# marcowus/forging-control

Hardware: AMD Instinct MI355X
Metric: rollout-steps/s (batch x horizon), fwd+bwd+AdamW step (higher is better)
Workload: dtype f32

## Files before the change

### forging-control_amd/csrc/fcr_common.h

```cpp
#pragma once
#include <hip/hip_runtime.h>
#include <stddef.h>
#include <stdint.h>

namespace fcr {

typedef float f32x4 __attribute__((ext_vector_type(4)));
typedef float f32x2 __attribute__((ext_vector_type(2)));

constexpr int kWave = 64;
constexpr int kTile = 16;
constexpr int kL = 10;
constexpr int kLayers = 3;
constexpr int kIn = 5;
constexpr int kOut = 4;
constexpr int kCtrlIn = 3;
constexpr int kMS = 13;
constexpr int kFnpStride = 8;
constexpr int kFwdWaves = 8;
constexpr int kBwdWaves = 8;
constexpr float kP1Max = 2.122366f;
constexpr float kP2Max = 1.036233f;

template <int HS>
// ... 9 lines not shown
    const float *fcb;
    const float *fnp;
    const float *wsc;
};

struct FwdArgs {
    int B, N;
    float alpha;
    const float *X, *u0, *states, *noise;
    float *cost, *command, *error, *prediction, *xhat_user, *xhat_ws, *loss_part;
    f32x4 *hseq;
    f32x4 *cseq;
    f32x2 *xw;
    unsigned long long *stamp;
    Packed p;
};

struct BwdArgs {
    int B, N, hidden;
    float alpha;
    const float *X, *states, *prediction, *xhat, *dloss;
    const f32x4 *hseq, *cseq;
    const f32x2 *xw;
    f32x4 *dseq;
    f32x2 *dxrow;
    float *g_u0;
    float *dv;
    unsigned long long *stamp;
    Packed p;
};
// ... 251 lines not shown
    return xor_sum_q(part);
}

__device__ __forceinline__ void grad_out5(float *part, int hidden, int k, int p, float s, float *gwi, float *gbi,
                                          float *gwo) {
    if (gwi) {
        const float v = 0.0f + s;
        if (p < 3) gwi[k * kCtrlIn + p] = v;
        else if (p == 3) gbi[k] = v;
        else gwo[k] = v;
    } else {
        part[((size_t)blockIdx.x * hidden + k) * 5 + p] = s;
    }
}

}
```

### forging-control_amd/csrc/fcr_f16.h

```cpp
#pragma once
#include "fcr_common.h"
#include "fcr_pack.h"

namespace fcr {

typedef _Float16 f16x8 __attribute__((ext_vector_type(8)));

__host__ __device__ constexpr bool tail_packed(int HS) { return 2 * HS - 8 * ((2 * HS + 7) / 8 - 1) == 2; }

template <int HS>
struct Geo16 {
    static constexpr int KB0 = (HS + 2 + 7) / 8;
    static constexpr int XBLK = HS >> 3;
    static constexpr int KB1 = (2 * HS + 7) / 8;
    static constexpr int KX1 = (HS + 7) / 8;
    static constexpr bool TAIL1 = tail_packed(HS);
    static constexpr int QF0 = HS * KB0 * 2;
    static constexpr int QH1 = HS * KB1;
    static constexpr int QF1 = QH1 + HS * (KB1 - (TAIL1 ? 1 : 0));
    static constexpr int FA0 = QF0 * kWave * 4, FA1 = QF1 * kWave * 4, FH1 = QH1 * kWave * 4;
    static constexpr int FNP = kMS * 4 * kFnpStride;
    static constexpr int FCP = kOut * HS * 4;
    static constexpr int MISC = FNP + FCP + 4;
    static constexpr int LDS_FWD = (FA1 + FA0 + MISC) * 4;
// ... 297 lines not shown
    const float d_o = 1.0f + __builtin_amdgcn_exp2f(__builtin_amdgcn_fmed3f(a[3], -1e30f, 126.0f));
    const float o = __builtin_amdgcn_rcpf(d_o);
    const float gi = g * i;
    const float cf = FIRST ? 0.0f : f * c_prev;
    const float tc = h * d_o;
    P = f32x4{fmaf(-h, tc, o), fmaf(-h, o, h), fmaf(-gi, i, gi), fmaf(-cf, f, cf)};
    Q = f32x2{fmaf(-gi, g, i), f};
}

inline size_t f16_fwd_bytes(int HS, int l) {
    const int KB = l == 0 ? (HS + 2 + 7) / 8 : (2 * HS + 7) / 8;
    const int lo_blocks = (l > 0 && tail_packed(HS)) ? KB - 1 : KB;
    return (size_t)HS * (KB + lo_blocks) * kWave * 16;
}

__device__ __forceinline__ float fwd16_weight(const PackArgs &a, int l, int unit, int gate, int s, int kq) {
    const int H = a.H, HS = a.HS;
    float v = 0.0f;
    if (unit < H) {
        const int grow = gate * H + unit;
        if (l == 0) {
            if (s < HS) {
                const int u = 4 * s + kq;
                if (u < H) v = a.whh[0][grow * H + u];
            } else if (s == HS) {
                v = a.wih[0][grow * kIn + kq] / a.wsc[kq];
            } else if (s == HS + 1 && kq == 0) {
                v = a.wih[0][grow * kIn + 4] / a.wsc[4];
            }
        } else if (s < HS) {
            const int u = 4 * s + kq;
            if (u < H) v = a.wih[l][grow * H + u];
        } else if (s < 2 * HS) {
            const int u = 4 * (s - HS) + kq;
            if (u < H) v = a.whh[l][grow * H + u];
        }
    }
    return v * (gate == 2 ? kTwoLog2e : kNegLog2e);
}

__device__ __forceinline__ void pack_fwd16_item(const PackArgs &a, int l, _Float16 *dst, int idx) {
    const int HS = a.HS;
    const int KB = l == 0 ? (HS + 2 + 7) / 8 : (2 * HS + 7) / 8;
    const bool tail = l > 0 && tail_packed(HS);
    const int KL = tail ? KB - 1 : KB;
    const int n = HS * KB * kWave * 8;
    if (idx >= n) return;
    const int j = idx & 7, lane = (idx >> 3) & 63, rk = idx >> 9;
    const int kb = rk % KB, r = rk / KB;
    const int rho = lane & 15, kq = lane >> 4;
    const int unit = 4 * r + (rho >> 2), gate = rho & 3;
    if (tail && kb == KB - 1) {
        _Float16 out = (_Float16)0.0f;
        if (j < 6) {
            const float v = fwd16_weight(a, l, unit, gate, 8 * kb + (j & 1), kq);
            const _Float16 hi = (_Float16)v;
            out = (j == 2 || j == 3) ? (_Float16)(v - (float)hi) : hi;
        }
        dst[((size_t)rk * kWave + lane) * 8 + j] = out;
        return;
    }
    const float v = fwd16_weight(a, l, unit, gate, 8 * kb + j, kq);
    const _Float16 hi = (_Float16)v;
    const _Float16 lo = (_Float16)(v - (float)hi);
    const size_t nq = (size_t)HS * KB;
    dst[((size_t)rk * kWave + lane) * 8 + j] = hi;
    dst[((nq + (size_t)r * KL + kb) * kWave + lane) * 8 + j] = lo;
}

}
```

### forging-control_amd/csrc/fcr_fwd.h

```cpp
#pragma once
#include "fcr_common.h"
#include "fcr_f16.h"

namespace fcr {

__device__ __forceinline__ void rot_left(float (&w)[kL]) {
    const float t0 = w[0];
#pragma unroll
    for (int k = 0; k < kL - 1; ++k) w[k] = w[k + 1];
    w[kL - 1] = t0;
}

struct Pace {
    unsigned turn;
};
__device__ __forceinline__ void pace_cell(Pace &p) {
    if (p.turn & 1) __builtin_amdgcn_s_setprio(1);
    else __builtin_amdgcn_s_setprio(0);
    p.turn ^= 1;
}

template <int HS, bool L0, bool FIRST, bool LP, int R0 = 0, int R1 = HS>
__device__ __forceinline__ void fwd16_cell(const float *__restrict__ lw, int lane, float x0, float x1,
                                           const float (&x)[HS], const float (&hp)[HS], float (&c)[HS],
// ... 293 lines not shown
        const float err = sq(xh0 - ref);
        const float con = relu(-xh1) + relu(-xh2) + relu(xh1 - kP1Max) + relu(xh2 - kP2Max);
        tot_sum += (err + cmd_j) + con;
        err_sum += err;
        cmd_sum += cmd_j;
    }
    const float cost = tot_sum / (float)N;
    if (valid && q == 0) {
        a.cost[b] = cost;
        a.command[b] = cmd_sum / (float)N;
        a.error[b] = err_sum / (float)N;
    }
    float part = (valid && q == 0) ? cost : 0.0f;
#pragma unroll
    for (int m = 1; m < 64; m <<= 1) part += __shfl_xor(part, m);
    if (lane == 0) a.loss_part[wave] = part;
#if FCR_STAMP
    if (lane == 0) {
        unsigned long long *o = a.stamp + (size_t)wave * 8;
        o[0] = st_head;
        o[1] = st_l0;
        o[2] = st_fill;
        o[3] = st_l2;
        o[4] = fstamp() - st_k0;
        o[5] = o[6] = o[7] = 0;
    }
#endif
}

}
```

### forging-control_amd/csrc/fcr_host.h

```cpp
#pragma once
#include <hip/hip_runtime.h>
#include <stdint.h>

#include <atomic>

#include "fcr.h"
#include "fcr_common.h"

namespace fcr {

int fail(int code, const char *fmt, ...) __attribute__((format(printf, 2, 3)));
int launch_check(const char *what);
int lds_attr(const void *fn, int bytes, std::atomic<unsigned long long> &done, const char *what);
extern std::atomic<int> g_small_max_batch, g_pipe_max_batch, g_pipe_sets;
extern std::atomic<long long> g_wide_keep_budget;

constexpr int kMaxSlots = 13;
constexpr int kMaxWideH = 2048;
inline bool is_wide(const fcr_dims *d) { return d->H > 4 * kMaxSlots; }
inline int slot_tier(int H) { return H <= 16 ? 4 : (H <= 32 ? 8 : 13); }
inline void note_kernels(fcr_options *o, int family) {
    if (o) o->kernels = family;
}

// ... 3 lines not shown
    size_t operator()(size_t bytes) {
        const size_t o = off;
        off += align_up(bytes);
        return o;
    }
};

struct PackedLayout {
    int HS;
    size_t fa[3], img[3], fcp, fcb, fnp, wsc, rng;
};
void take_packed(Arena &take, PackedLayout &P, bool with_backward);
Packed packed_ptrs(const PackedLayout &P, char *base);
int launch_range(const fcr_dims *d, const float *states, const float *u0, const float *noise, const float *fcw,
                 const float *fcb, float *part, float *wsc, hipStream_t s);
int launch_pack_all(const fcr_weights *w, int H, int CH, const PackedLayout &P, bool with_backward, char *base,
                    unsigned *clear, int nclear, hipStream_t s);
int launch_pack_ctrl(const fcr_weights *w, int CH, float *fcp, float *fcbo, float *fnp, hipStream_t s);
int launch_loss_reduce(const float *part, int n, int B, float *loss, hipStream_t s);
int launch_ctrl_grads(const fcr_dims *d, const float *X, const float *xhat, const float *dv, const float *fnp, float *part,
                      int ctrl_blocks, float *g_w_inp, float *g_b_inp, float *g_w_out, hipStream_t s);
int launch_grad_reduce(const float *part, int blocks, int hidden, float *g_w_inp, float *g_b_inp, float *g_w_out,
                       hipStream_t s);
int launch_grad_reduce_many(const float *part, int blocks, int hidden, int n_models, float *g_w_inp, float *g_b_inp,
                            float *g_w_out, hipStream_t s);
int pipe_max_sets();
size_t rollout_workspace(const fcr_dims *d, int with_backward);
int rollout_forward(const fcr_dims *d, fcr_options *opts, const fcr_weights *w, const float *X, const float *u0,
                    const float *states, const float *noise, float *loss, float *cost, float *command, float *error,
                    float *prediction, float *xhat, int with_backward, char *base, hipStream_t s);
int rollout_backward(const fcr_dims *d, fcr_options *opts, const float *X, const float *states, const float *prediction,
                     const float *dloss, float *g_u0, float *g_w_inp, float *g_b_inp, float *g_w_out, char *base,
// ... 41 lines not shown
```

### forging-control_amd/csrc/fcr_img.h

```cpp
#pragma once
#include "fcr_common.h"
#include "fcr_f16.h"
#include "fcr_pack.h"

namespace fcr {

__host__ __device__ constexpr int img_units(int kb) { return kb > 2 ? 32 : 16; }
__host__ __device__ constexpr int img_tile_units(int U) { return U == 32 ? 536 : 268; }
__host__ __device__ constexpr int img_row_start(int m, int U) {
    return U == 32 ? 33 * m + (m >= 8 ? 8 : 0)
                   : 33 * (m % 4 + 4 * (m / 8)) + (m >= 8 ? 4 : 0) + 16 * ((m / 4) % 2);
}
__host__ __device__ constexpr int img_unit(int kb, int q, int h0, int U) { return q * (U / 4) + 2 * kb + h0; }

template <int HS, bool L0>
struct Img {
    static constexpr int NSL = L0 ? HS + 2 : 2 * HS;
    static constexpr int KB = (NSL + 7) / 8;
    static constexpr int U = img_units(KB);
    static constexpr int TILE = 8 * img_tile_units(U);
    static constexpr int HALF = HS * TILE;
    static constexpr int BYTES = (2 * HALF + 1023) / 1024 * 1024;
    static constexpr int NB = (NSL + 3) / 4;
    static constexpr int KBB = (HS + 1) / 2;
};

inline int img_kb(int HS, int l) { return ((l == 0 ? HS + 2 : 2 * HS) + 7) / 8; }
inline size_t img_bytes(int HS, int l) {
    const int U = img_units(img_kb(HS, l));
    return ((size_t)2 * HS * 8 * img_tile_units(U) + 1023) / 1024 * 1024;
}
inline int img_pack_threads(int HS, int l) { return 16 * HS * 4 * img_units(img_kb(HS, l)); }

__device__ __forceinline__ void pack_img_item(const PackArgs &a, int l, _Float16 *dst, int idx) {
    const int H = a.H, HS = a.HS;
    const int nsl = l == 0 ? HS + 2 : 2 * HS;
    const int kbn = (nsl + 7) / 8;
    const int U = img_units(kbn), TU = img_tile_units(U);
    const int cols = 4 * U, rows = 16 * HS;
    if (idx >= rows * cols) return;
    const int col = idx % cols, R = idx / cols;
    const int slot = R >> 4, m = R & 15;
    const int unit = 4 * slot + (m >> 2), gate = m & 3;
    const int sg = (col >> 5) * 8 + (col & 7), grp = (col >> 3) & 3;
    auto weight = [&](int s) {
        float v = 0.0f;
        if (unit < H && s < nsl) {
            const int grow = gate * H + unit;
            if (l == 0) {
                if (s < HS) {
                    const int u = 4 * s + grp;
                    if (u < H) v = a.whh[0][grow * H + u];
                } else if (s == HS) {
                    v = a.wih[0][grow * kIn + grp] / a.wsc[grp];
                } else if (grp == 0) {
                    v = a.wih[0][grow * kIn + 4] / a.wsc[4];
                }
            } else if (s < HS) {
                const int u = 4 * s + grp;
                if (u < H) v = a.wih[l][grow * H + u];
            } else {
                const int u = 4 * (s - HS) + grp;
                if (u < H) v = a.whh[l][grow * H + u];
            }
        }
        return v * (gate == 2 ? kTwoLog2e : kNegLog2e);
    };
    _Float16 hi, lo;
    const int jt = sg - 8 * (kbn - 1);
    if (l > 0 && tail_packed(HS) && jt >= 2 && jt < 6) {
        const float v = weight(8 * (kbn - 1) + (jt & 1));
// ... 48 lines not shown
```

### forging-control_amd/csrc/fcr_pack.h

```cpp
#pragma once
#include "fcr_common.h"

namespace fcr {

struct PackArgs {
    int H, HS, CH;
    const float *wih[3], *whh[3], *fcw, *fcb, *cwi, *cbi, *cwo;
    float *fcp, *fcbo, *fnp;
    const float *wsc;
};

constexpr int kRangeBlocks = 128;
constexpr int kRangeThreads = 256;
__device__ __forceinline__ void range_final_wave(const float *__restrict__ part, int nblk,
                                                 const float *__restrict__ fcw, const float *__restrict__ fcb,
                                                 int H, float *wsc, int lane) {
    float mc[kIn];
#pragma unroll
    for (int c = 0; c < kIn; ++c) {
        float m = 0.0f;
        for (int i = lane; i < nblk; i += 64) m = fmaxf(m, part[i * 8 + c]);
#pragma unroll
        for (int o = 32; o > 0; o >>= 1) m = fmaxf(m, __shfl_xor(m, o));
        mc[c] = m;
// ... 14 lines not shown
#pragma unroll
                for (int j = 0; j < 8; ++j) v[j] = w[k + j];
#pragma unroll
                for (int j = 0; j < 8; ++j) s += fabsf(v[j]);
            }
            for (; k < H; ++k) s += fabsf(w[k]);
            m += s;
        } else {
            m = fmaxf(m, 1.0f);
        }
        if (isfinite(m) && m >= 16384.0f) sc = __builtin_amdgcn_ldexpf(1.0f, 14 - __builtin_amdgcn_frexp_expf(m));
    }
    wsc[lane] = sc;
}

__device__ __forceinline__ void pack_misc_item(const PackArgs &a, int idx) {
    const int H = a.H, HS = a.HS;
    const int nfc = kOut * HS * 4;
    if (idx < nfc) {
        const int q = idx & 3, r = (idx >> 2) % HS, o = (idx >> 2) / HS;
        const int u = 4 * r + q;
        a.fcp[idx] = u < H ? a.fcw[o * H + u] : 0.0f;
    }
    if (idx < kOut) a.fcbo[idx] = a.fcb[idx];
    const int nf = kMS * 4 * kFnpStride;
    if (idx < nf) {
        const int p = idx % kFnpStride, q = (idx / kFnpStride) & 3, m = idx / (kFnpStride * 4);
        const int k = 4 * m + q;
        float v = 0.0f;
        if (k < a.CH) {
// ... 13 lines not shown
```

### forging-control_amd/csrc/fcr_rollout.hip

```cpp
#include <hip/hip_runtime.h>
#include <stdint.h>

#include <atomic>

#include "fcr.h"
#include "fcr_bwd.h"
#include "fcr_common.h"
#include "fcr_fwd.h"
#include "fcr_host.h"
#include "fcr_img.h"
#include "fcr_pack.h"
#include "fcr_pipe.h"
#include "fcr_shared_kernels.h"
#include "fcr_small.h"
#include "fcr_sur.h"
#include "fcr_lstm_rollout.h"

namespace fcr {
namespace {

struct Layout : PackedLayout {
    int nw, nw_pad;
    size_t xhat, dv, loss_part, fnn_part, hseq, cseq, xw, dseq, dxrow, stamp, total;
    size_t pipe_flags, pipe_rows;
    int ctrl_blocks;
};

constexpr int kPipeMaxGroups = 32;

Layout make_layout(const fcr_dims *d, int with_backward) {
    Layout L{};
    L.HS = slot_tier(d->H);
    L.nw = (d->B + kTile - 1) / kTile;
    constexpr int kPad = kFwdWaves > kBwdWaves ? kFwdWaves : kBwdWaves;
    L.nw_pad = (L.nw + kPad - 1) / kPad * kPad;
    Arena take;
    const int HS = L.HS;
    take_packed(take, L, with_backward != 0);
    L.xhat = take(sizeof(float) * (size_t)d->B * d->N * kOut);
    L.loss_part = take(sizeof(float) * L.nw_pad);
    L.dv = take(sizeof(float) * (size_t)d->B * d->N);
    L.ctrl_blocks = (int)(((long long)d->B * d->N + kCtrlItems - 1) / kCtrlItems);
    L.fnn_part = take(sizeof(float) * (size_t)L.ctrl_blocks * d->ctrl_hidden * 5);
// ... 132 lines not shown
    hipLaunchKernelGGL((fcr_sbwd_kernel<HS>), dim3(L.nw), dim3(Small<HS>::NQ * kWave), lds, s, ba);
    return launch_check("fcr_sbwd_kernel");
}

enum { kPackFwd16 = 0, kPackImg = 1, kPackMisc = 2 };
struct PackJob {
    int kind, l, blocks;
    _Float16 *dst;
};
struct PackAllArgs {
    PackArgs a;
    int njobs;
    PackJob job[2 * kLayers + 1];
    unsigned *clear;
    int nclear;
};
__global__ __launch_bounds__(256) void pack_all_kernel(PackAllArgs p) {
    if (p.clear && blockIdx.x == 0)
        for (int i = (int)threadIdx.x; i < p.nclear; i += 256) p.clear[i] = 0u;
    int b = blockIdx.x, j = 0;
    while (j + 1 < p.njobs && b >= p.job[j].blocks) b -= p.job[j++].blocks;
    const int idx = b * 256 + (int)threadIdx.x;
    const PackJob &jb = p.job[j];
    if (jb.kind == kPackFwd16) pack_fwd16_item(p.a, jb.l, jb.dst, idx);
    else if (jb.kind == kPackImg) pack_img_item(p.a, jb.l, jb.dst, idx);
    else pack_misc_item(p.a, idx);
}
}

void take_packed(Arena &take, PackedLayout &P, bool with_backward) {
    const int HS = P.HS;
    for (int l = 0; l < kLayers; ++l) P.fa[l] = take(f16_fwd_bytes(HS, l));
    if (with_backward)
        for (int l = 0; l < kLayers; ++l) P.img[l] = take(img_bytes(HS, l));
    P.fcp = take(sizeof(float) * kOut * HS * 4);
    P.fcb = take(sizeof(float) * kOut);
    P.fnp = take(sizeof(float) * kMS * 4 * kFnpStride);
    P.wsc = take(sizeof(float) * 8);
    P.rng = take(sizeof(float) * 8 * kRangeBlocks);
}

int launch_pack_all(const fcr_weights *w, int H, int CH, const PackedLayout &P, bool with_backward, char *base,
                    unsigned *clear, int nclear, hipStream_t s) {
    PackAllArgs pk{};
    PackArgs &pa = pk.a;
    pa.H = H;
    pa.HS = P.HS;
    pa.CH = CH;
    for (int l = 0; l < kLayers; ++l) {
        pa.wih[l] = w->w_ih[l];
        pa.whh[l] = w->w_hh[l];
    }
    pa.fcw = w->fc_w;
    pa.fcb = w->fc_b;
    if (CH) {
        pa.cwi = w->ctrl_w_inp;
        pa.cbi = w->ctrl_b_inp;
        pa.cwo = w->ctrl_w_out;
    }
    pa.fcp = (float *)(base + P.fcp);
    pa.fcbo = (float *)(base + P.fcb);
    pa.fnp = (float *)(base + P.fnp);
    pa.wsc = (const float *)(base + P.wsc);
    pk.clear = clear;
    pk.nclear = nclear;
    for (int l = 0; l < kLayers; ++l) {
        const int nf = P.HS * (l == 0 ? (P.HS + 2 + 7) / 8 : (2 * P.HS + 7) / 8) * kWave * 8;
        pk.job[pk.njobs++] = PackJob{kPackFwd16, l, (nf + 255) / 256, (_Float16 *)(base + P.fa[l])};
        if (with_backward)
            pk.job[pk.njobs++] = PackJob{kPackImg, l, (img_pack_threads(P.HS, l) + 255) / 256, (_Float16 *)(base + P.img[l])};
    }
    pk.job[pk.njobs++] = PackJob{kPackMisc, 0, 2, nullptr};
    int blocks = 0;
    for (int j = 0; j < pk.njobs; ++j) blocks += pk.job[j].blocks;
    hipLaunchKernelGGL(pack_all_kernel, dim3(blocks), dim3(256), 0, s, pk);
    return launch_check("pack_all_kernel");
}

int launch_pack_ctrl(const fcr_weights *w, int CH, float *fcp, float *fcbo, float *fnp, hipStream_t s) {
    PackArgs pa{};
// ... 30 lines not shown
    const size_t rows = (size_t)d->B * (d->N > kL ? d->N : kL);
    if (rows <= 16 * kRangeThreads) {
        hipLaunchKernelGGL(range_partial_kernel, dim3(1), dim3(kRangeThreads), 0, s, states, u0, noise, d->B, d->N,
                           part, fcw, fcb, d->H, wsc);
        return launch_check("range_partial_kernel");
    }
    hipLaunchKernelGGL(range_partial_kernel, dim3(kRangeBlocks), dim3(kRangeThreads), 0, s, states, u0, noise, d->B,
                       d->N, part, nullptr, nullptr, 0, nullptr);
    int rc = launch_check("range_partial_kernel");
    if (rc) return rc;
    hipLaunchKernelGGL(range_final_kernel, dim3(1), dim3(64), 0, s, (const float *)part, kRangeBlocks, fcw, fcb, d->H,
                       wsc);
    return launch_check("range_final_kernel");
}

int launch_ctrl_grads(const fcr_dims *d, const float *X, const float *xhat, const float *dv, const float *fnp, float *part,
                      int ctrl_blocks, float *g_w_inp, float *g_b_inp, float *g_w_out, hipStream_t s) {
    const bool one = ctrl_blocks == 1;
    hipLaunchKernelGGL(ctrl_grad_kernel, dim3(ctrl_blocks), dim3(kCtrlBlock), 0, s, X, xhat, dv, fnp, d->B, d->N,
                       d->ctrl_hidden, part, one ? g_w_inp : nullptr, one ? g_b_inp : nullptr, one ? g_w_out : nullptr);
    if (const int rc = launch_check("ctrl_grad_kernel")) return rc;
    if (one) return FCR_OK;
    return launch_grad_reduce(part, ctrl_blocks, d->ctrl_hidden, g_w_inp, g_b_inp, g_w_out, s);
}

int launch_grad_reduce(const float *part, int blocks, int hidden, float *g_w_inp, float *g_b_inp, float *g_w_out,
                       hipStream_t s) {
    hipLaunchKernelGGL(grad_reduce_kernel, dim3(hidden * 5), dim3(256), 0, s, part, blocks, hidden, g_w_inp, g_b_inp,
                       g_w_out);
    return launch_check("grad_reduce_kernel");
// ... 8 lines not shown
                            float *g_w_out, hipStream_t s) {
    hipLaunchKernelGGL(grad_reduce_many_kernel, dim3(hidden * 5, n_models), dim3(256), 0, s, part, blocks, hidden, g_w_inp,
                       g_b_inp, g_w_out);
    return launch_check("grad_reduce_many_kernel");
}

int pipe_max_sets() { return Pipe<13>::MAX_SETS; }

size_t rollout_workspace(const fcr_dims *d, int with_backward) { return make_layout(d, with_backward).total; }

int rollout_forward(const fcr_dims *d, fcr_options *opts, const fcr_weights *w, const float *X, const float *u0,
                    const float *states, const float *noise, float *loss, float *cost, float *command, float *error,
                    float *prediction, float *xhat, int with_backward, char *base, hipStream_t s) {
    int rc;
    const Layout L = make_layout(d, with_backward);
    if ((rc = launch_range(d, states, u0, noise, w->fc_w, w->fc_b, (float *)(base + L.rng), (float *)(base + L.wsc), s)))
        return rc;
    const bool flags = L.nw <= kPipeMaxGroups;
    if ((rc = launch_pack_all(w, d->H, d->ctrl_hidden, L, with_backward != 0, base,
                              flags ? (unsigned *)(base + L.pipe_flags) : nullptr, flags ? L.nw * kPipeFlags : 0, s)))
        return rc;

    FwdArgs fa{};
    fa.B = d->B;
    fa.N = d->N;
    fa.alpha = d->alpha;
    fa.X = X;
    fa.u0 = u0;
    fa.states = states;
    fa.noise = noise;
    fa.cost = cost;
    fa.command = command;
    fa.error = error;
    fa.prediction = prediction;
    fa.xhat_user = xhat;
    fa.xhat_ws = (float *)(base + L.xhat);
    fa.loss_part = (float *)(base + L.loss_part);
    fa.hseq = (f32x4 *)(base + L.hseq);
    fa.cseq = with_backward ? (f32x4 *)(base + L.cseq) : nullptr;
    fa.xw = with_backward ? (f32x2 *)(base + L.xw) : nullptr;
    fa.p = packed_ptrs(L, base);
#if FCR_STAMP
    fa.stamp = (unsigned long long *)(base + L.stamp) + (size_t)L.nw_pad * 8;
#endif
    const bool small = use_small(d, L, opts);
    note_kernels(opts, small ? FCR_KERNELS_SMALL : FCR_KERNELS_FUSED);
    const bool piped = small && use_pipe(d, L, opts);
    if (piped) {
        PipeArgs pa = pipe_args(L, base);
        pa.loss = loss;
        const int S = pipe_sets(d, L, Pipe<13>::MAX_SETS, 2);
        if (L.HS == 8) rc = with_backward ? launch_pfwd_s<8, true>(fa, pa, L, S, s) : launch_pfwd_s<8, false>(fa, pa, L, S, s);
        else rc = with_backward ? launch_pfwd_s<13, true>(fa, pa, L, S, s) : launch_pfwd_s<13, false>(fa, pa, L, S, s);
    } else if (small) {
        if (L.HS == 8) rc = with_backward ? launch_sfwd_t<8, true>(fa, L, s) : launch_sfwd_t<8, false>(fa, L, s);
        else rc = with_backward ? launch_sfwd_t<13, true>(fa, L, s) : launch_sfwd_t<13, false>(fa, L, s);
    } else {
        switch (L.HS) {
            case 4: rc = launch_fwd<4>(fa, L, d->precision == FCR_PRECISION_F16, s); break;
            case 8: rc = launch_fwd<8>(fa, L, d->precision == FCR_PRECISION_F16, s); break;
            case 13: rc = launch_fwd<13>(fa, L, d->precision == FCR_PRECISION_F16, s); break;
            default: rc = fail(FCR_EUNSUPPORTED, "H=%d", d->H);
        }
    }
    if (rc) return rc;
    if (piped) return FCR_OK;
    return launch_loss_reduce(fa.loss_part, small ? L.nw : L.nw_pad, d->B, loss, s);
}

int rollout_backward(const fcr_dims *d, fcr_options *opts, const float *X, const float *states, const float *prediction,
                     const float *dloss, float *g_u0, float *g_w_inp, float *g_b_inp, float *g_w_out, char *base,
                     hipStream_t s) {
    int rc;
    const Layout L = make_layout(d, 1);
    BwdArgs ba{};
    ba.B = d->B;
    ba.N = d->N;
    ba.hidden = d->ctrl_hidden;
    ba.alpha = d->alpha;
    ba.X = X;
    ba.states = states;
    ba.prediction = prediction;
// ... 89 lines not shown
    const int HS = slot_tier(d->H);
    return !is_wide(d) && (HS == 8 || HS == 13);
}

size_t many_workspace(const fcr_dims *d, int n_models, int with_backward) {
    return make_many(d, n_models, with_backward).total;
}

int many_forward(const fcr_dims *d, int M, const fcr_weights *w, const float *X, const float *u0, const float *states,
                 const float *noise, float *loss, float *cost, float *command, float *error, float *prediction,
                 float *xhat, int with_backward, char *base, hipStream_t s) {
    int rc;
    const ManyLayout L = make_many(d, M, with_backward);
    fcr_dims all = *d;
    all.B = M * d->B;
    if ((rc = launch_range(&all, states, u0, noise, w->fc_w, w->fc_b, (float *)(base + L.rng), (float *)(base + L.wsc), s)))
        return rc;
    if ((rc = launch_pack_all(w, d->H, 0, L, with_backward != 0, base, nullptr, 0, s))) return rc;
    constexpr int nf = kMS * 4 * kFnpStride;
    hipLaunchKernelGGL(pack_fnp_many_kernel, dim3((nf + 255) / 256, M), dim3(256), 0, s, w->ctrl_w_inp, w->ctrl_b_inp,
                       w->ctrl_w_out, d->ctrl_hidden, (float *)(base + L.fnp_many));
    if ((rc = launch_check("pack_fnp_many_kernel"))) return rc;

    FwdArgs fa{};
    fa.B = d->B;
    fa.N = d->N;
    fa.alpha = d->alpha;
    fa.X = X;
    fa.u0 = u0;
    fa.states = states;
    fa.noise = noise;
    fa.cost = cost;
    fa.command = command;
// ... 155 lines not shown
    int rc = launch_check("sur_bwd_kernel");
    if (rc) return rc;
    if ((rc = sur_wgrad_t<HS, false>(a, L, 2, part, g_w_ih[2], g_w_hh[2], s))) return rc;
    if ((rc = sur_wgrad_t<HS, false>(a, L, 1, part, g_w_ih[1], g_w_hh[1], s))) return rc;
    return sur_wgrad_t<HS, true>(a, L, 0, part, g_w_ih[0], g_w_hh[0], s);
}

}

size_t sur_workspace(const fcr_dims *d, int with_backward) { return make_sur(d, with_backward).total; }

int sur_forward(const fcr_dims *d, const fcr_weights *w, const float *x, float *y, int with_backward, char *base,
                hipStream_t s) {
    const SurLayout L = make_sur(d, with_backward);
    int rc;
    if ((rc = launch_range(d, x, x, nullptr, w->fc_w, w->fc_b, (float *)(base + L.rng), (float *)(base + L.wsc), s)))
        return rc;
    if ((rc = launch_pack_all(w, d->H, 0, L, with_backward != 0, base, nullptr, 0, s))) return rc;
    SurArgs a = sur_args(d, L, base);
    a.x = x;
    a.y = y;
    switch (L.HS) {
        case 4: return sur_forward_t<4>(a, L, with_backward != 0, s);
        case 8: return sur_forward_t<8>(a, L, with_backward != 0, s);
        default: return sur_forward_t<13>(a, L, with_backward != 0, s);
    }
}

int sur_backward(const fcr_dims *d, const float *dy, float *const *g_w_ih, float *const *g_w_hh, float *g_fc_w,
                 float *g_fc_b, float *g_x, char *base, hipStream_t s) {
    const SurLayout L = make_sur(d, 1);
    SurArgs a = sur_args(d, L, base);
    a.dy = dy;
// ... 62 lines not shown
    a.g3 = gain ? gain[3] : 1.0f;
    a.xhat = xhat;
    a.hseq = (f32x4 *)(base + L.hseq);
    a.p = packed_ptrs(L, base);
    float *part = (float *)(base + L.rpart), *wsc = (float *)(base + L.wsc);
    const size_t rows = (size_t)d->B * (d->N > kL ? d->N : kL);
    const LroRangeArgs rg{a.g0, a.g1, a.g2, a.g3, w->fc_w, w->fc_b, w->w_ih[0], d->H, wsc};
    const bool one = rows <= 16 * kRangeThreads;
    hipLaunchKernelGGL(lro_range_partial_kernel, dim3(one ? 1 : kRangeBlocks), dim3(kRangeThreads), 0, s, window0, cmd,
                       noise, d->B, d->N, part, one ? 1 : 0, rg);
    if ((rc = launch_check("lro_range_partial_kernel"))) return rc;
    if (!one) {
        hipLaunchKernelGGL(lro_range_final_kernel, dim3(1), dim3(64), 0, s, (const float *)part, kRangeBlocks, rg);
        if ((rc = launch_check("lro_range_final_kernel"))) return rc;
    }
    if ((rc = launch_pack_all(w, d->H, 0, L, false, base, nullptr, 0, s))) return rc;
    switch (L.HS) {
        case 4: return launch_lro_t<4>(a, L, s);
        case 8: return launch_lro_t<8>(a, L, s);
        default: return launch_lro_t<13>(a, L, s);
    }
}

}

#if FCR_STAMP
extern "C" {
size_t fcr_debug_stamp_offset(const fcr_dims *d) { return fcr::make_layout(d, 1).stamp; }
size_t fcr_debug_dseq_offset(const fcr_dims *d) { return fcr::make_layout(d, 1).dseq; }
size_t fcr_debug_dxrow_offset(const fcr_dims *d) { return fcr::make_layout(d, 1).dxrow; }
}
// ... 2 lines not shown
```

### forging-control_amd/csrc/fcr_shared_kernels.h

```cpp
#pragma once
#include "fcr_f16.h"
#include "fcr_img.h"
#include "fcr_pack.h"

namespace fcr {

__global__ __launch_bounds__(64) void range_final_kernel(const float *__restrict__ part, int nblk,
                                                         const float *__restrict__ fcw,
                                                         const float *__restrict__ fcb, int H, float *wsc) {
    range_final_wave(part, nblk, fcw, fcb, H, wsc, threadIdx.x);
}

__global__ __launch_bounds__(kRangeThreads) void range_partial_kernel(const float *__restrict__ states,
                                                                      const float *__restrict__ u0,
                                                                      const float *__restrict__ noise, int B, int N,
                                                                      float *part, const float *fcw = nullptr,
                                                                      const float *fcb = nullptr, int H = 0,
                                                                      float *wsc = nullptr) {
    __shared__ float red[kIn][kRangeThreads];
    float m0 = 0.0f, m1 = 0.0f, m2 = 0.0f, m3 = 0.0f, m4 = 0.0f;
    const size_t stride = (size_t)gridDim.x * blockDim.x, tid0 = (size_t)blockIdx.x * blockDim.x + threadIdx.x;
    const size_t rows = (size_t)B * kL;
    for (size_t r = tid0; r < rows; r += stride) {
        const float *p = states + r * kIn;
        m0 = fmaxf(m0, fabsf(p[0]));
        m1 = fmaxf(m1, fabsf(p[1]));
        m2 = fmaxf(m2, fabsf(p[2]));
        m3 = fmaxf(m3, fabsf(p[3]));
        m4 = fmaxf(m4, fabsf(p[4]));
    }
    for (size_t b = tid0; b < (size_t)B; b += stride) m4 = fmaxf(m4, fabsf(u0[b]));
    if (noise)
        for (size_t r = tid0; r < (size_t)B * N; r += stride) {
            const float *p = noise + r * kOut;
            m0 = fmaxf(m0, fabsf(p[0]));
            m1 = fmaxf(m1, fabsf(p[1]));
            m2 = fmaxf(m2, fabsf(p[2]));
            m3 = fmaxf(m3, fabsf(p[3]));
        }
    red[0][threadIdx.x] = m0;
    red[1][threadIdx.x] = m1;
    red[2][threadIdx.x] = m2;
    red[3][threadIdx.x] = m3;
    red[4][threadIdx.x] = m4;
    __syncthreads();
    for (int w = kRangeThreads / 2; w > 0; w >>= 1) {
        if ((int)threadIdx.x < w)
            for (int c = 0; c < kIn; ++c) red[c][threadIdx.x] = fmaxf(red[c][threadIdx.x], red[c][threadIdx.x + w]);
        __syncthreads();
    }
    if (threadIdx.x < kIn) part[blockIdx.x * 8 + threadIdx.x] = red[threadIdx.x][0];
    if (wsc) {
        __syncthreads();
        if (threadIdx.x < 64) range_final_wave(part, 1, fcw, fcb, H, wsc, threadIdx.x);
    }
}

__global__ void pack_misc_kernel(PackArgs a) { pack_misc_item(a, blockIdx.x * blockDim.x + threadIdx.x); }

__device__ __forceinline__ void loss_reduce_block(const float *part, int nw, int B, float *loss) {
    __shared__ float red[256];
    float s = 0.0f;
    for (int i = threadIdx.x; i < nw; i += blockDim.x) s += part[i];
    red[threadIdx.x] = s;
    __syncthreads();
    for (int w = 128; w > 0; w >>= 1) {
        if ((int)threadIdx.x < w) red[threadIdx.x] += red[threadIdx.x + w];
        __syncthreads();
    }
    if (threadIdx.x == 0) loss[0] = red[0] / (float)B;
}
__global__ void loss_reduce_kernel(const float *part, int nw, int B, float *loss) { loss_reduce_block(part, nw, B, loss); }
__global__ void loss_reduce_many_kernel(const float *part, int gpm, int B, float *loss) {
    loss_reduce_block(part + (size_t)blockIdx.x * gpm, gpm, B, loss + blockIdx.x);
}

__device__ __forceinline__ void ctrl_grad_block(const float *X, const float *xhat, const float *dv, const float *fnp,
                                                int B, int N, int hidden, float *part, float *gwi, float *gbi,
                                                float *gwo) {
    __shared__ float sx0[kCtrlItems], sx3[kCtrlItems], sref[kCtrlItems], sdv[kCtrlItems];
    __shared__ float red[kCtrlBlock / kWave][64][5];
    const long long items = (long long)B * N;
    const long long i0 = (long long)blockIdx.x * kCtrlItems;
    const int n = (int)((items - i0) < kCtrlItems ? (items - i0) : kCtrlItems);
    for (int i = threadIdx.x; i < n; i += blockDim.x) {
// ... 1 lines not shown
        const int bb = (int)(it / N);
        sx0[i] = xhat[it * kOut + 0];
        sx3[i] = xhat[it * kOut + 3];
        sref[i] = X[(size_t)bb * kCtrlIn + 2];
        sdv[i] = dv[it];
    }
    __syncthreads();
    const int lane = threadIdx.x & 63, w = threadIdx.x >> 6;
    const int k = lane;
    float W0 = 0.0f, W1 = 0.0f, W2 = 0.0f, bk = 0.0f, wo = 0.0f;
    if (k < hidden) {
        const float *p = fnp + ((k >> 2) * 4 + (k & 3)) * kFnpStride;
        W0 = p[0]; W1 = p[1]; W2 = p[2]; bk = p[3]; wo = p[4];
    }
    float g0 = 0.0f, g1 = 0.0f, g2 = 0.0f, g3 = 0.0f, g4 = 0.0f;
    for (int i = w; i < n; i += kCtrlBlock / kWave) {
        const float a = sx0[i], b3 = sx3[i], r = sref[i], d = sdv[i];
        const float z = W0 * a + W1 * b3 + W2 * r + bk;
        const float dz = z > 0.0f ? d * wo : 0.0f;
        g0 += dz * a;
        g1 += dz * b3;
        g2 += dz * r;
        g3 += dz;
        g4 += d * (z > 0.0f ? z : 0.0f);
    }
    red[w][lane][0] = g0; red[w][lane][1] = g1; red[w][lane][2] = g2; red[w][lane][3] = g3; red[w][lane][4] = g4;
    __syncthreads();
    if (w == 0 && k < hidden) {
#pragma unroll
        for (int p = 0; p < 5; ++p) {
// ... 53 lines not shown
    const int idx = blockIdx.x * blockDim.x + threadIdx.x;
    constexpr int nf = kMS * 4 * kFnpStride;
    if (idx >= nf) return;
    const size_t m = blockIdx.y;
    const int p = idx % kFnpStride, q = (idx / kFnpStride) & 3, k = 4 * (idx / (kFnpStride * 4)) + q;
    float v = 0.0f;
    if (k < CH) {
        if (p < 3) v = cwi[(m * CH + k) * kCtrlIn + p];
        else if (p == 3) v = cbi[m * CH + k];
        else if (p == 4) v = cwo[m * CH + k];
    }
    fnp[m * nf + idx] = v;
}

__global__ void pack_fwd16_kernel(PackArgs a, int l, _Float16 *dst) {
    pack_fwd16_item(a, l, dst, blockIdx.x * blockDim.x + threadIdx.x);
}
__global__ void pack_img_kernel(PackArgs a, int l, _Float16 *dst) {
    pack_img_item(a, l, dst, blockIdx.x * blockDim.x + threadIdx.x);
}

}
```

Baseline: 118.9 million.

## Fuse range finalization into pack kernel and loss reduction into forward kernel

Drops the separate range-final launch by having the pack kernel's blocks that need input scales recompute them from the range partials. Drops the separate loss-reduce launch by using an atomic last-block-arrives counter in the forward kernel, with agent-scope stores and loads for the partials. The range partial loop is unrolled by four and the control-gradient loop gets an unroll pragma. This cuts kernel launches and host-side gaps per step. In exchange it adds redundant per-block range reduction, an atomic counter that must be reset correctly, and a tail serialization in the last block.

```diff
diff --git a/forging-control_amd/csrc/fcr_common.h b/forging-control_amd/csrc/fcr_common.h
--- a/forging-control_amd/csrc/fcr_common.h
+++ b/forging-control_amd/csrc/fcr_common.h
@@ -47,6 +47,8 @@
     f32x2 *xw;
     unsigned long long *stamp;
     Packed p;
+    unsigned *loss_ctr;
+    float *loss;
 };
 
 struct BwdArgs {
@@ -328,4 +330,38 @@
     }
 }
 
-}
+__device__ __forceinline__ void st_agent(float *p, float v) {
+    __hip_atomic_store(p, v, __ATOMIC_RELAXED, __HIP_MEMORY_SCOPE_AGENT);
+}
+__device__ __forceinline__ float ld_agent(const float *p) {
+    return __hip_atomic_load(p, __ATOMIC_RELAXED, __HIP_MEMORY_SCOPE_AGENT);
+}
+__device__ __forceinline__ bool last_block_arrives(unsigned *ctr, unsigned nblk, unsigned *flag, int tid) {
+    asm volatile("s_waitcnt vmcnt(0)" ::: "memory");
+    __syncthreads();
+    if (tid == 0) {
+        const unsigned t = __hip_atomic_fetch_add(ctr, 1u, __ATOMIC_RELAXED, __HIP_MEMORY_SCOPE_AGENT);
+        const bool last = t + 1u == nblk;
+        if (last) __hip_atomic_store(ctr, 0u, __ATOMIC_RELAXED, __HIP_MEMORY_SCOPE_AGENT);
+        *flag = last ? 1u : 0u;
+    }
+    __syncthreads();
+    return *flag != 0u;
+}
+
+template <bool AGENT>
+__device__ __forceinline__ void loss_sum_256(const float *part, int nw, int B, float *loss, float *red, int t) {
+    if (t < 256) {
+        float s = 0.0f;
+        for (int i = t; i < nw; i += 256) s += AGENT ? ld_agent(part + i) : part[i];
+        red[t] = s;
+    }
+    __syncthreads();
+    for (int w = 128; w > 0; w >>= 1) {
+        if (t < w) red[t] += red[t + w];
+        __syncthreads();
+    }
+    if (t == 0) loss[0] = red[0] / (float)B;
+}
+
+}
diff --git a/forging-control_amd/csrc/fcr_f16.h b/forging-control_amd/csrc/fcr_f16.h
--- a/forging-control_amd/csrc/fcr_f16.h
+++ b/forging-control_amd/csrc/fcr_f16.h
@@ -335,7 +335,8 @@
     return (size_t)HS * (KB + lo_blocks) * kWave * 16;
 }
 
-__device__ __forceinline__ float fwd16_weight(const PackArgs &a, int l, int unit, int gate, int s, int kq) {
+__device__ __forceinline__ float fwd16_weight(const PackArgs &a, const float *wsc, int l, int unit, int gate, int s,
+                                              int kq) {
     const int H = a.H, HS = a.HS;
     float v = 0.0f;
     if (unit < H) {
@@ -345,9 +346,9 @@
                 const int u = 4 * s + kq;
                 if (u < H) v = a.whh[0][grow * H + u];
             } else if (s == HS) {
-                v = a.wih[0][grow * kIn + kq] / a.wsc[kq];
+                v = a.wih[0][grow * kIn + kq] / wsc[kq];
             } else if (s == HS + 1 && kq == 0) {
-                v = a.wih[0][grow * kIn + 4] / a.wsc[4];
+                v = a.wih[0][grow * kIn + 4] / wsc[4];
             }
         } else if (s < HS) {
             const int u = 4 * s + kq;
@@ -360,7 +361,7 @@
     return v * (gate == 2 ? kTwoLog2e : kNegLog2e);
 }
 
-__device__ __forceinline__ void pack_fwd16_item(const PackArgs &a, int l, _Float16 *dst, int idx) {
+__device__ __forceinline__ void pack_fwd16_item(const PackArgs &a, const float *wsc, int l, _Float16 *dst, int idx) {
     const int HS = a.HS;
     const int KB = l == 0 ? (HS + 2 + 7) / 8 : (2 * HS + 7) / 8;
     const bool tail = l > 0 && tail_packed(HS);
@@ -374,14 +375,14 @@
     if (tail && kb == KB - 1) {
         _Float16 out = (_Float16)0.0f;
         if (j < 6) {
-            const float v = fwd16_weight(a, l, unit, gate, 8 * kb + (j & 1), kq);
+            const float v = fwd16_weight(a, wsc, l, unit, gate, 8 * kb + (j & 1), kq);
             const _Float16 hi = (_Float16)v;
             out = (j == 2 || j == 3) ? (_Float16)(v - (float)hi) : hi;
         }
         dst[((size_t)rk * kWave + lane) * 8 + j] = out;
         return;
     }
-    const float v = fwd16_weight(a, l, unit, gate, 8 * kb + j, kq);
+    const float v = fwd16_weight(a, wsc, l, unit, gate, 8 * kb + j, kq);
     const _Float16 hi = (_Float16)v;
     const _Float16 lo = (_Float16)(v - (float)hi);
     const size_t nq = (size_t)HS * KB;
diff --git a/forging-control_amd/csrc/fcr_fwd.h b/forging-control_amd/csrc/fcr_fwd.h
--- a/forging-control_amd/csrc/fcr_fwd.h
+++ b/forging-control_amd/csrc/fcr_fwd.h
@@ -331,7 +331,7 @@
     float part = (valid && q == 0) ? cost : 0.0f;
 #pragma unroll
     for (int m = 1; m < 64; m <<= 1) part += __shfl_xor(part, m);
-    if (lane == 0) a.loss_part[wave] = part;
+    if (lane == 0) st_agent(a.loss_part + wave, part);
 #if FCR_STAMP
     if (lane == 0) {
         unsigned long long *o = a.stamp + (size_t)wave * 8;
@@ -343,6 +343,10 @@
         o[5] = o[6] = o[7] = 0;
     }
 #endif
-}
-
-}
+    const int tid = (wave - (int)blockIdx.x * kFwdWaves) * kWave +
+                    (int)__builtin_amdgcn_mbcnt_hi(~0u, __builtin_amdgcn_mbcnt_lo(~0u, 0u));
+    if (last_block_arrives(a.loss_ctr, gridDim.x, (unsigned *)lw, tid))
+        loss_sum_256<true>(a.loss_part, (int)gridDim.x * kFwdWaves, a.B, a.loss, lw + 64, tid);
+}
+
+}
diff --git a/forging-control_amd/csrc/fcr_host.h b/forging-control_amd/csrc/fcr_host.h
--- a/forging-control_amd/csrc/fcr_host.h
+++ b/forging-control_amd/csrc/fcr_host.h
@@ -41,8 +41,10 @@
 Packed packed_ptrs(const PackedLayout &P, char *base);
 int launch_range(const fcr_dims *d, const float *states, const float *u0, const float *noise, const float *fcw,
                  const float *fcb, float *part, float *wsc, hipStream_t s);
+int launch_range_partials(const fcr_dims *d, const float *states, const float *u0, const float *noise, const float *fcw,
+                          const float *fcb, float *part, float *wsc, int *nrng, hipStream_t s);
 int launch_pack_all(const fcr_weights *w, int H, int CH, const PackedLayout &P, bool with_backward, char *base,
-                    unsigned *clear, int nclear, hipStream_t s);
+                    unsigned *clear, int nclear, unsigned *ctr, int nctr, int nrng, hipStream_t s);
 int launch_pack_ctrl(const fcr_weights *w, int CH, float *fcp, float *fcbo, float *fnp, hipStream_t s);
 int launch_loss_reduce(const float *part, int n, int B, float *loss, hipStream_t s);
 int launch_ctrl_grads(const fcr_dims *d, const float *X, const float *xhat, const float *dv, const float *fnp, float *part,
diff --git a/forging-control_amd/csrc/fcr_img.h b/forging-control_amd/csrc/fcr_img.h
--- a/forging-control_amd/csrc/fcr_img.h
+++ b/forging-control_amd/csrc/fcr_img.h
@@ -32,7 +32,7 @@
 }
 inline int img_pack_threads(int HS, int l) { return 16 * HS * 4 * img_units(img_kb(HS, l)); }
 
-__device__ __forceinline__ void pack_img_item(const PackArgs &a, int l, _Float16 *dst, int idx) {
+__device__ __forceinline__ void pack_img_item(const PackArgs &a, const float *wsc, int l, _Float16 *dst, int idx) {
     const int H = a.H, HS = a.HS;
     const int nsl = l == 0 ? HS + 2 : 2 * HS;
     const int kbn = (nsl + 7) / 8;
@@ -52,9 +52,9 @@
                     const int u = 4 * s + grp;
                     if (u < H) v = a.whh[0][grow * H + u];
                 } else if (s == HS) {
-                    v = a.wih[0][grow * kIn + grp] / a.wsc[grp];
+                    v = a.wih[0][grow * kIn + grp] / wsc[grp];
                 } else if (grp == 0) {
-                    v = a.wih[0][grow * kIn + 4] / a.wsc[4];
+                    v = a.wih[0][grow * kIn + 4] / wsc[4];
                 }
             } else if (s < HS) {
                 const int u = 4 * s + grp;
diff --git a/forging-control_amd/csrc/fcr_pack.h b/forging-control_amd/csrc/fcr_pack.h
--- a/forging-control_amd/csrc/fcr_pack.h
+++ b/forging-control_amd/csrc/fcr_pack.h
@@ -52,6 +52,32 @@
     wsc[lane] = sc;
 }
 
+constexpr int kRangeFusedBlocks = kRangeBlocks * 8 / kIn;
+__device__ __forceinline__ void range_final_block(const float *__restrict__ part, int nblk,
+                                                  const float *__restrict__ fcw, const float *__restrict__ fcb,
+                                                  int H, float *wsc, float *lds) {
+    const int t = threadIdx.x, c = t & 7;
+    constexpr int kRounds = (kRangeFusedBlocks + 31) / 32;
+    float v[kRounds];
+#pragma unroll
+    for (int k = 0; k < kRounds; ++k) {
+        const int i = (t >> 3) + 32 * k;
+        v[k] = (c < kIn && i < nblk) ? part[i * kIn + c] : 0.0f;
+    }
+    const float w = t < kOut * H ? fcw[t] : 0.0f;
+    const float b = t < kOut ? fcb[t] : 0.0f;
+    float m = 0.0f;
+#pragma unroll
+    for (int k = 0; k < kRounds; ++k) m = fmaxf(m, v[k]);
+    lds[t] = m;
+    float *fc = lds + 256;
+    if (t < kOut * H) fc[t] = w;
+    if (t < kOut) fc[kOut * H + t] = b;
+    __syncthreads();
+    if (t < 64) range_final_wave(lds, 32, fc, fc + kOut * H, H, wsc, t);
+    __syncthreads();
+}
+
 __device__ __forceinline__ void pack_misc_item(const PackArgs &a, int idx) {
     const int H = a.H, HS = a.HS;
     const int nfc = kOut * HS * 4;
diff --git a/forging-control_amd/csrc/fcr_rollout.hip b/forging-control_amd/csrc/fcr_rollout.hip
--- a/forging-control_amd/csrc/fcr_rollout.hip
+++ b/forging-control_amd/csrc/fcr_rollout.hip
@@ -27,6 +27,8 @@
 };
 
 constexpr int kPipeMaxGroups = 32;
+constexpr int kCounters = 8, kCtrWord = 16;
+unsigned *counters(const PackedLayout &P, char *base) { return (unsigned *)(base + P.wsc) + kCtrWord; }
 
 Layout make_layout(const fcr_dims *d, int with_backward) {
     Layout L{};
@@ -189,16 +191,29 @@
     PackJob job[2 * kLayers + 1];
     unsigned *clear;
     int nclear;
+    unsigned *ctr;
+    int nctr;
+    const float *rng;
+    int nrng;
+    float *wsc_out;
 };
 __global__ __launch_bounds__(256) void pack_all_kernel(PackAllArgs p) {
+    __shared__ float s_wsc[8], s_rng[256 + kOut * 52 + kOut];
     if (p.clear && blockIdx.x == 0)
         for (int i = (int)threadIdx.x; i < p.nclear; i += 256) p.clear[i] = 0u;
+    if (p.ctr && blockIdx.x == 0 && (int)threadIdx.x < p.nctr) p.ctr[threadIdx.x] = 0u;
     int b = blockIdx.x, j = 0;
     while (j + 1 < p.njobs && b >= p.job[j].blocks) b -= p.job[j++].blocks;
     const int idx = b * 256 + (int)threadIdx.x;
     const PackJob &jb = p.job[j];
-    if (jb.kind == kPackFwd16) pack_fwd16_item(p.a, jb.l, jb.dst, idx);
-    else if (jb.kind == kPackImg) pack_img_item(p.a, jb.l, jb.dst, idx);
+    const float *wsc = p.a.wsc;
+    if (p.rng && (blockIdx.x == 0 || (jb.kind != kPackMisc && jb.l == 0))) {
+        range_final_block(p.rng, p.nrng, p.a.fcw, p.a.fcb, p.a.H, s_wsc, s_rng);
+        if (blockIdx.x == 0 && threadIdx.x < 8) p.wsc_out[threadIdx.x] = s_wsc[threadIdx.x];
+        wsc = s_wsc;
+    }
+    if (jb.kind == kPackFwd16) pack_fwd16_item(p.a, wsc, jb.l, jb.dst, idx);
+    else if (jb.kind == kPackImg) pack_img_item(p.a, wsc, jb.l, jb.dst, idx);
     else pack_misc_item(p.a, idx);
 }
 }
@@ -212,11 +227,12 @@
     P.fcb = take(sizeof(float) * kOut);
     P.fnp = take(sizeof(float) * kMS * 4 * kFnpStride);
     P.wsc = take(sizeof(float) * 8);
+    static_assert(kIn * kRangeFusedBlocks <= 8 * kRangeBlocks, "the fused range pass's partials fit the same slab");
     P.rng = take(sizeof(float) * 8 * kRangeBlocks);
 }
 
 int launch_pack_all(const fcr_weights *w, int H, int CH, const PackedLayout &P, bool with_backward, char *base,
-                    unsigned *clear, int nclear, hipStream_t s) {
+                    unsigned *clear, int nclear, unsigned *ctr, int nctr, int nrng, hipStream_t s) {
     PackAllArgs pk{};
     PackArgs &pa = pk.a;
     pa.H = H;
@@ -239,6 +255,11 @@
     pa.wsc = (const float *)(base + P.wsc);
     pk.clear = clear;
     pk.nclear = nclear;
+    pk.ctr = ctr;
+    pk.nctr = nctr;
+    pk.rng = nrng ? (const float *)(base + P.rng) : nullptr;
+    pk.nrng = nrng;
+    pk.wsc_out = (float *)(base + P.wsc);
     for (int l = 0; l < kLayers; ++l) {
         const int nf = P.HS * (l == 0 ? (P.HS + 2 + 7) / 8 : (2 * P.HS + 7) / 8) * kWave * 8;
         pk.job[pk.njobs++] = PackJob{kPackFwd16, l, (nf + 255) / 256, (_Float16 *)(base + P.fa[l])};
@@ -299,6 +320,19 @@
     return launch_check("range_final_kernel");
 }
 
+int launch_range_partials(const fcr_dims *d, const float *states, const float *u0, const float *noise, const float *fcw,
+                          const float *fcb, float *part, float *wsc, int *nrng, hipStream_t s) {
+    const size_t rows = (size_t)d->B * (d->N > kL ? d->N : kL);
+    *nrng = 0;
+    if (rows <= 16 * kRangeThreads) return launch_range(d, states, u0, noise, fcw, fcb, part, wsc, s);
+    const size_t want = (rows + 4 * kRangeThreads - 1) / (4 * kRangeThreads);
+    const int blocks = want < (size_t)kRangeFusedBlocks ? (int)want : kRangeFusedBlocks;
+    hipLaunchKernelGGL(range_partial_kernel, dim3(blocks), dim3(kRangeThreads), 0, s, states, u0, noise, d->B, d->N, part,
+                       nullptr, nullptr, 0, nullptr, kIn);
+    *nrng = blocks;
+    return launch_check("range_partial_kernel");
+}
+
 int launch_ctrl_grads(const fcr_dims *d, const float *X, const float *xhat, const float *dv, const float *fnp, float *part,
                       int ctrl_blocks, float *g_w_inp, float *g_b_inp, float *g_w_out, hipStream_t s) {
     const bool one = ctrl_blocks == 1;
@@ -337,11 +371,14 @@
                     float *prediction, float *xhat, int with_backward, char *base, hipStream_t s) {
     int rc;
     const Layout L = make_layout(d, with_backward);
-    if ((rc = launch_range(d, states, u0, noise, w->fc_w, w->fc_b, (float *)(base + L.rng), (float *)(base + L.wsc), s)))
+    int nrng = 0;
+    if ((rc = launch_range_partials(d, states, u0, noise, w->fc_w, w->fc_b, (float *)(base + L.rng), (float *)(base + L.wsc),
+                                    &nrng, s)))
         return rc;
     const bool flags = L.nw <= kPipeMaxGroups;
     if ((rc = launch_pack_all(w, d->H, d->ctrl_hidden, L, with_backward != 0, base,
-                              flags ? (unsigned *)(base + L.pipe_flags) : nullptr, flags ? L.nw * kPipeFlags : 0, s)))
+                              flags ? (unsigned *)(base + L.pipe_flags) : nullptr, flags ? L.nw * kPipeFlags : 0,
+                              counters(L, base), kCounters, nrng, s)))
         return rc;
 
     FwdArgs fa{};
@@ -363,6 +400,8 @@
     fa.cseq = with_backward ? (f32x4 *)(base + L.cseq) : nullptr;
     fa.xw = with_backward ? (f32x2 *)(base + L.xw) : nullptr;
     fa.p = packed_ptrs(L, base);
+    fa.loss_ctr = counters(L, base);
+    fa.loss = loss;
 #if FCR_STAMP
     fa.stamp = (unsigned long long *)(base + L.stamp) + (size_t)L.nw_pad * 8;
 #endif
@@ -387,8 +426,8 @@
         }
     }
     if (rc) return rc;
-    if (piped) return FCR_OK;
-    return launch_loss_reduce(fa.loss_part, small ? L.nw : L.nw_pad, d->B, loss, s);
+    if (piped || !small) return FCR_OK;
+    return launch_loss_reduce(fa.loss_part, L.nw, d->B, loss, s);
 }
 
 int rollout_backward(const fcr_dims *d, fcr_options *opts, const float *X, const float *states, const float *prediction,
@@ -508,9 +547,11 @@
     const ManyLayout L = make_many(d, M, with_backward);
     fcr_dims all = *d;
     all.B = M * d->B;
-    if ((rc = launch_range(&all, states, u0, noise, w->fc_w, w->fc_b, (float *)(base + L.rng), (float *)(base + L.wsc), s)))
+    int nrng = 0;
+    if ((rc = launch_range_partials(&all, states, u0, noise, w->fc_w, w->fc_b, (float *)(base + L.rng),
+                                    (float *)(base + L.wsc), &nrng, s)))
         return rc;
-    if ((rc = launch_pack_all(w, d->H, 0, L, with_backward != 0, base, nullptr, 0, s))) return rc;
+    if ((rc = launch_pack_all(w, d->H, 0, L, with_backward != 0, base, nullptr, 0, nullptr, 0, nrng, s))) return rc;
     constexpr int nf = kMS * 4 * kFnpStride;
     hipLaunchKernelGGL(pack_fnp_many_kernel, dim3((nf + 255) / 256, M), dim3(256), 0, s, w->ctrl_w_inp, w->ctrl_b_inp,
                        w->ctrl_w_out, d->ctrl_hidden, (float *)(base + L.fnp_many));
@@ -696,9 +737,11 @@
                 hipStream_t s) {
     const SurLayout L = make_sur(d, with_backward);
     int rc;
-    if ((rc = launch_range(d, x, x, nullptr, w->fc_w, w->fc_b, (float *)(base + L.rng), (float *)(base + L.wsc), s)))
+    int nrng = 0;
+    if ((rc = launch_range_partials(d, x, x, nullptr, w->fc_w, w->fc_b, (float *)(base + L.rng), (float *)(base + L.wsc),
+                                    &nrng, s)))
         return rc;
-    if ((rc = launch_pack_all(w, d->H, 0, L, with_backward != 0, base, nullptr, 0, s))) return rc;
+    if ((rc = launch_pack_all(w, d->H, 0, L, with_backward != 0, base, nullptr, 0, nullptr, 0, nrng, s))) return rc;
     SurArgs a = sur_args(d, L, base);
     a.x = x;
     a.y = y;
@@ -791,7 +834,7 @@
         hipLaunchKernelGGL(lro_range_final_kernel, dim3(1), dim3(64), 0, s, (const float *)part, kRangeBlocks, rg);
         if ((rc = launch_check("lro_range_final_kernel"))) return rc;
     }
-    if ((rc = launch_pack_all(w, d->H, 0, L, false, base, nullptr, 0, s))) return rc;
+    if ((rc = launch_pack_all(w, d->H, 0, L, false, base, nullptr, 0, nullptr, 0, 0, s))) return rc;
     switch (L.HS) {
         case 4: return launch_lro_t<4>(a, L, s);
         case 8: return launch_lro_t<8>(a, L, s);
diff --git a/forging-control_amd/csrc/fcr_shared_kernels.h b/forging-control_amd/csrc/fcr_shared_kernels.h
--- a/forging-control_amd/csrc/fcr_shared_kernels.h
+++ b/forging-control_amd/csrc/fcr_shared_kernels.h
@@ -16,12 +16,28 @@
                                                                       const float *__restrict__ noise, int B, int N,
                                                                       float *part, const float *fcw = nullptr,
                                                                       const float *fcb = nullptr, int H = 0,
-                                                                      float *wsc = nullptr) {
+                                                                      float *wsc = nullptr, int pstride = 8) {
     __shared__ float red[kIn][kRangeThreads];
     float m0 = 0.0f, m1 = 0.0f, m2 = 0.0f, m3 = 0.0f, m4 = 0.0f;
     const size_t stride = (size_t)gridDim.x * blockDim.x, tid0 = (size_t)blockIdx.x * blockDim.x + threadIdx.x;
     const size_t rows = (size_t)B * kL;
-    for (size_t r = tid0; r < rows; r += stride) {
+    size_t r = tid0;
+    for (; r + 3 * stride < rows; r += 4 * stride) {
+        float v[4][kIn];
+#pragma unroll
+        for (int k = 0; k < 4; ++k)
+#pragma unroll
+            for (int c = 0; c < kIn; ++c) v[k][c] = states[(r + k * stride) * kIn + c];
+#pragma unroll
+        for (int k = 0; k < 4; ++k) {
+            m0 = fmaxf(m0, fabsf(v[k][0]));
+            m1 = fmaxf(m1, fabsf(v[k][1]));
+            m2 = fmaxf(m2, fabsf(v[k][2]));
+            m3 = fmaxf(m3, fabsf(v[k][3]));
+            m4 = fmaxf(m4, fabsf(v[k][4]));
+        }
+    }
+    for (; r < rows; r += stride) {
         const float *p = states + r * kIn;
         m0 = fmaxf(m0, fabsf(p[0]));
         m1 = fmaxf(m1, fabsf(p[1]));
@@ -49,7 +65,7 @@
             for (int c = 0; c < kIn; ++c) red[c][threadIdx.x] = fmaxf(red[c][threadIdx.x], red[c][threadIdx.x + w]);
         __syncthreads();
     }
-    if (threadIdx.x < kIn) part[blockIdx.x * 8 + threadIdx.x] = red[threadIdx.x][0];
+    if (threadIdx.x < kIn) part[blockIdx.x * pstride + threadIdx.x] = red[threadIdx.x][0];
     if (wsc) {
         __syncthreads();
         if (threadIdx.x < 64) range_final_wave(part, 1, fcw, fcb, H, wsc, threadIdx.x);
@@ -60,15 +76,7 @@
 
 __device__ __forceinline__ void loss_reduce_block(const float *part, int nw, int B, float *loss) {
     __shared__ float red[256];
-    float s = 0.0f;
-    for (int i = threadIdx.x; i < nw; i += blockDim.x) s += part[i];
-    red[threadIdx.x] = s;
-    __syncthreads();
-    for (int w = 128; w > 0; w >>= 1) {
-        if ((int)threadIdx.x < w) red[threadIdx.x] += red[threadIdx.x + w];
-        __syncthreads();
-    }
-    if (threadIdx.x == 0) loss[0] = red[0] / (float)B;
+    loss_sum_256<false>(part, nw, B, loss, red, threadIdx.x);
 }
 __global__ void loss_reduce_kernel(const float *part, int nw, int B, float *loss) { loss_reduce_block(part, nw, B, loss); }
 __global__ void loss_reduce_many_kernel(const float *part, int gpm, int B, float *loss) {
@@ -100,6 +108,7 @@
         W0 = p[0]; W1 = p[1]; W2 = p[2]; bk = p[3]; wo = p[4];
     }
     float g0 = 0.0f, g1 = 0.0f, g2 = 0.0f, g3 = 0.0f, g4 = 0.0f;
+#pragma unroll 4
     for (int i = w; i < n; i += kCtrlBlock / kWave) {
         const float a = sx0[i], b3 = sx3[i], r = sref[i], d = sdv[i];
         const float z = W0 * a + W1 * b3 + W2 * r + bk;
@@ -183,10 +192,10 @@
 }
 
 __global__ void pack_fwd16_kernel(PackArgs a, int l, _Float16 *dst) {
-    pack_fwd16_item(a, l, dst, blockIdx.x * blockDim.x + threadIdx.x);
+    pack_fwd16_item(a, a.wsc, l, dst, blockIdx.x * blockDim.x + threadIdx.x);
 }
 __global__ void pack_img_kernel(PackArgs a, int l, _Float16 *dst) {
-    pack_img_item(a, l, dst, blockIdx.x * blockDim.x + threadIdx.x);
-}
-
-}
+    pack_img_item(a, a.wsc, l, dst, blockIdx.x * blockDim.x + threadIdx.x);
+}
+
+}
```

New measurement: 119.2 million, median of 6. Within noise of the previous version (+0.3%).
